# GavinLynch04/FastSelect

Hardware: AMD Instinct MI355X
Metric: feature-scores/sec (n*p/s) MultiSURF fp32 (higher is better)
Workload: dtype u16 pass 1, fp32 pass 2 (fp64 accumulation)

## Files before the change

fastselect_amd/csrc/fs_colsort.hip:

```cpp
#include <hip/hip_runtime.h>

#include <cstdlib>

#include <rocprim/block/block_radix_sort.hpp>
#include <rocprim/device/device_segmented_radix_sort.hpp>

#include "fs_internal.h"

namespace fs {
namespace gpu {

namespace {

constexpr double kEpsFx = 16777216.0;
constexpr int kCsThreads = 1024;
constexpr int kCsMaxIpt = 24;

__device__ __forceinline__ uint32_t cs_col_q(const uint32_t* __restrict__ xqT, int64_t c,
                                             int64_t i, int64_t n_pad, int q16) {
  return q16 ? (xqT[(c >> 1) * n_pad + i] >> ((c & 1) * 16)) & 0xFFFFu : xqT[c * n_pad + i];
}

__device__ __forceinline__ int32_t cs_fx(float eps) { return __float2int_rn(eps * 16777216.0f); }

__device__ __forceinline__ uint32_t cs_key(uint32_t q, int32_t fx, int s) {
  const uint32_t fr = (uint32_t)(((1 << 23) - fx) >> (24 - s));
  const uint32_t m = (1u << s) - 1u;
  return (q << s) | (fr < m ? fr : m);
}

__device__ __forceinline__ float cs_term(long long e, long long pos, long long n, long long P,
                                         long long T) {
  return (float)((double)(e * (2 * pos - n) - 2 * P + T) / kEpsFx);
}

__device__ __forceinline__ uint32_t cs_eq12_of_fx(int32_t fx) {
  const int32_t u = fx + (1 << 23);
  return (uint32_t)(u < 0 ? 0 : (u >= (1 << 24) ? 4095 : (u >> 12)));
}

__device__ __forceinline__ long long cs_block_scan(long long v, long long* wsum,
                                                   long long& total) {
  const int lane = threadIdx.x & 63, wave = threadIdx.x >> 6;
  long long x = v;
#pragma unroll
  for (int o = 1; o < 64; o <<= 1) {
    const long long t = __shfl_up(x, o);
    if (lane >= o) x += t;
  }
  if (lane == 63) wsum[wave] = x;
  __syncthreads();
  long long pre = 0, tot = 0;
#pragma unroll
  for (int w = 0; w < kCsThreads / 64; w++) {
    const long long s = wsum[w];
    pre += w < wave ? s : 0;
    tot += s;
  }
  __syncthreads();
  total = tot;
  return pre + x - v;
}

constexpr int kHistShift = 44;
constexpr int kMaxBinFill = 64;
constexpr uint32_t kPureEmpty = 0x7FFFFFFFu, kMixed = 0x80000000u;

__device__ __forceinline__ unsigned long long cs_code(int32_t fx) {
  return (1ull << kHistShift) + (unsigned long long)(uint32_t)(fx + (1 << 23));
}
__device__ __forceinline__ void cs_decode(unsigned long long v, long long& cnt, long long& esum) {
  cnt = (long long)(v >> kHistShift);
  esum = (long long)(v & ((1ull << kHistShift) - 1ull)) - (cnt << 23);
}

template <int IPT>
__global__ __launch_bounds__(kCsThreads) void k_colsort_full(const uint32_t* __restrict__ xqT,
                                                             int64_t n, int64_t n_pad, int s,
                                                             int q16, int64_t c_lo,
                                                             const int* __restrict__ crowded,
                                                             float* __restrict__ epsT) {
  using Sort = rocprim::block_radix_sort<uint32_t, kCsThreads, IPT, uint16_t>;
  __shared__ typename Sort::storage_type st;
  __shared__ long long wsum[kCsThreads / 64];
  if (!crowded[blockIdx.x]) return;
  const int64_t c = c_lo + blockIdx.x;
  float* __restrict__ e = epsT + c * n_pad;
  const int base = threadIdx.x * IPT;
  uint32_t key[IPT];
  uint16_t idx[IPT];
#pragma unroll
  for (int k = 0; k < IPT; k++) {
    const int i = base + k;
    key[k] = i < n ? cs_key(cs_col_q(xqT, c, i, n_pad, q16), cs_fx(e[i]), s) : 0xFFFFFFFFu;
    idx[k] = (uint16_t)i;
  }
  Sort().sort(key, idx, st);
  long long ef[IPT], loc = 0;
#pragma unroll
  for (int k = 0; k < IPT; k++) {
    ef[k] = base + k < n ? cs_fx(e[idx[k]]) : 0;
    loc += ef[k];
  }
  long long T;
  long long P = cs_block_scan(loc, wsum, T);
#pragma unroll
  for (int k = 0; k < IPT; k++) {
    const int pos = base + k;
    if (pos < n) e[idx[k]] = cs_term(ef[k], pos, n, P, T);
    P += ef[k];
  }
}

template <int IPT, int BB>
struct ColbinSmem {
  static constexpr int kBins = 1 << BB;
  unsigned long long hist[kBins];
  alignas(16) uint32_t seg[(kCsThreads * IPT > kBins ? kCsThreads * IPT : kBins) + 4];
  uint32_t starts[(kCsThreads * IPT + 31) / 32];
  uint32_t skip[(kCsThreads * IPT + 31) / 32];
  uint32_t binskip[kBins / 32];
  long long wsum[kCsThreads / 64];
  int max_fill;
};

#define FS_OPAQUE(v) asm volatile("" : "+v"(v))

__device__ __forceinline__ int32_t cs_pack(int d, int ds) { return ds * 256 + (d + 128); }
__device__ __forceinline__ void cs_unpack(int32_t r, int& d, int& ds) {
  d = (r & 255) - 128;
  ds = r >> 8;
}

template <int IPT, int BB>
__global__ __launch_bounds__(kCsThreads) void k_colsort(const uint32_t* __restrict__ xqT,
                                                        int64_t n, int64_t n_pad, int s, int q16,
                                                        int64_t c_lo, int* __restrict__ crowded,
                                                        float* __restrict__ epsT) {
  __shared__ ColbinSmem<IPT, BB> sm;
  constexpr int kBins = 1 << BB, kBinShift = 32 - BB;
  constexpr int kWords = (kCsThreads * IPT + 31) / 32;
  static_assert(sizeof(ColbinSmem<IPT, BB>) <= 160 * 1024, "k_colsort: LDS");
  const int tid = threadIdx.x;
  const int64_t c = c_lo + blockIdx.x;
  float* __restrict__ e = epsT + c * n_pad;
  const int nn = (int)n;
  uint32_t key[IPT];
  int32_t fx[IPT];
  for (int b = tid; b < kBins; b += kCsThreads) {
    sm.hist[b] = 0ull;
    sm.seg[b] = kPureEmpty;
  }
  for (int w = tid; w < kWords; w += kCsThreads) {
    sm.starts[w] = 0u;
    sm.skip[w] = 0u;
  }
  if (tid < kBins / 32) sm.binskip[tid] = 0u;
  if (tid == 0) sm.max_fill = 0;
  const __amdgpu_buffer_rsrc_t qbuf = __builtin_amdgcn_make_buffer_rsrc(
      (void*)(xqT + (q16 ? (c >> 1) : c) * n_pad), (short)0, nn * 4, 0x00020000);
  const __amdgpu_buffer_rsrc_t ebuf =
      __builtin_amdgcn_make_buffer_rsrc((void*)e, (short)0, nn * 4, 0x00020000);
  const int voff = tid * 4;
  const uint32_t qsh = q16 ? (uint32_t)(c & 1) * 16u : 0u;
  const uint32_t qmask = q16 ? 0xFFFFu : 0xFFFFFFFFu;
#pragma unroll
  for (int k = 0; k < IPT; k++) {
    key[k] = __builtin_amdgcn_raw_buffer_load_b32(qbuf, voff, kCsThreads * 4 * k, 0);
    fx[k] = (int32_t)__builtin_amdgcn_raw_buffer_load_b32(ebuf, voff, kCsThreads * 4 * k, 0);
  }
#pragma unroll
  for (int k = 0; k < IPT; k++) {
    fx[k] = cs_fx(__int_as_float(fx[k]));
    key[k] = cs_key((key[k] >> qsh) & qmask, fx[k], s);
  }
  __syncthreads();
#pragma unroll
  for (int k = 0; k < IPT; k++) {
    if (tid + kCsThreads * k >= nn) continue;
    const int b = (int)(key[k] >> kBinShift);
    atomicAdd(&sm.hist[b], cs_code(fx[k]));
    const uint32_t kl = key[k] & ((1u << kBinShift) - 1u);
    const uint32_t old = atomicCAS(&sm.seg[b], kPureEmpty, kl);
    if (old != kPureEmpty && (old & ((1u << kBinShift) - 1u)) != kl) atomicOr(&sm.seg[b], kMixed);
  }
  __syncthreads();
  constexpr int kPer = kBins / kCsThreads;
  unsigned long long run = 0;
  uint32_t skip_bits = 0;
  int fill = 0;
#pragma unroll
  for (int q = 0; q < kPer; q++) {
    const unsigned long long v = sm.hist[tid * kPer + q];
    const bool mixed = (sm.seg[tid * kPer + q] & kMixed) != 0u;
    run += v;
    if (mixed) fill = max(fill, (int)(v >> kHistShift));
    else skip_bits |= 1u << q;
  }
  long long tot_packed;
  const unsigned long long pre = (unsigned long long)cs_block_scan((long long)run, sm.wsum, tot_packed);
  unsigned long long ex = pre;
#pragma unroll 1
  for (int q = 0; q < kPer; q++) {
    const unsigned long long v = sm.hist[tid * kPer + q];
    const uint32_t lo = (uint32_t)(ex >> kHistShift);
    const uint32_t m = (uint32_t)(v >> kHistShift);
    const bool skip = ((skip_bits >> q) & 1u) != 0u;
    sm.hist[tid * kPer + q] = ex;
    ex += v;
    if (m != 0u) {
      atomicOr(&sm.starts[lo >> 5], 1u << (lo & 31));
      if (skip) {
        const uint32_t hi = lo + m;
        for (uint32_t w = lo >> 5; w <= (hi - 1) >> 5; w++) {
          const uint32_t a = w == (lo >> 5) ? (lo & 31) : 0u;
          const uint32_t z = w == ((hi - 1) >> 5) ? ((hi - 1) & 31) : 31u;
          const uint32_t bits = (0xFFFFFFFFu >> (31u - z)) & (0xFFFFFFFFu << a);
          atomicOr(&sm.skip[w], bits);
        }
      }
    }
  }
  atomicOr(&sm.binskip[(tid * kPer) >> 5], skip_bits << ((tid * kPer) & 31));
  atomicMax(&sm.max_fill, fill);
  __syncthreads();
  const bool crowd = sm.max_fill > kMaxBinFill;
  if (tid == 0) crowded[blockIdx.x] = crowd ? 1 : 0;
  if (crowd) return;
  long long n_all, T;
  cs_decode((unsigned long long)tot_packed, n_all, T);
  int t3 = tid;
  FS_OPAQUE(t3);
#pragma unroll
  for (int k = 0; k < IPT; k++) {
    FS_OPAQUE(key[k]);
    FS_OPAQUE(fx[k]);
    const uint32_t b = key[k] >> kBinShift;
    uint32_t pos = 0xFFFFu;
    if (t3 + kCsThreads * k < nn) {
      const uint32_t at = (uint32_t)(atomicAdd(&sm.hist[b], 1ull << kHistShift) >> kHistShift);
      if (!((sm.binskip[b >> 5] >> (b & 31)) & 1u)) {
        pos = at;
        sm.seg[pos] = ((key[k] & ((1u << kBinShift) - 1u)) << 12) | cs_eq12_of_fx(fx[k]);
      }
    }
    key[k] = (b << 16) | pos;
    FS_OPAQUE(key[k]);
    __builtin_amdgcn_sched_barrier(0);
  }
  __syncthreads();
  int32_t res[IPT];
  int t4 = tid;
  FS_OPAQUE(t4);
#pragma unroll
  for (int k = 0; k < IPT; k++) {
    const int j = t4 + kCsThreads * k;
    res[k] = 0;
    if (j >= nn || ((sm.skip[j >> 5] >> (j & 31)) & 1u)) continue;
    int w = j >> 5;
    uint32_t bits = sm.starts[w] & (0xFFFFFFFFu >> (31 - (j & 31)));
    while (bits == 0u) bits = sm.starts[--w];
    const int lo = w * 32 + 31 - __clz(bits);
    int hi = nn;
    w = j >> 5;
    bits = (j & 31) == 31 ? 0u : sm.starts[w] & (0xFFFFFFFFu << ((j & 31) + 1));
    while (bits == 0u && ++w < kWords && w * 32 < nn) bits = sm.starts[w];
    if (bits != 0u) hi = min(nn, w * 32 + __ffs(bits) - 1);
    const uint32_t v = sm.seg[j];
    const uint32_t mine_lo = v & ~0xFFFu, mine_hi = v | 0xFFFu;
    uint32_t a_lt = 0u, a_le = 0u, a_all = 0u;
    for (int jj = lo; jj < hi; jj++) {
      const uint32_t u = sm.seg[jj];
      const uint32_t wv = (u & 0xFFFu) | (1u << 20);
      a_lt += u < mine_lo ? wv : 0u;
      a_le += u <= mine_hi ? wv : 0u;
      a_all += wv;
    }
    const int l = (int)(a_lt >> 20), sl = (int)(a_lt & 0xFFFFFu);
    const int g = (int)(a_all >> 20) - (int)(a_le >> 20);
    const int sg = (int)(a_all & 0xFFFFFu) - (int)(a_le & 0xFFFFFu);
    res[k] = cs_pack(l - g, sl - sg);
    __builtin_amdgcn_sched_barrier(0);
  }
  __syncthreads();
#pragma unroll
  for (int k = 0; k < IPT; k++) {
    const int j = t4 + kCsThreads * k;
    if (j < nn && !((sm.skip[j >> 5] >> (j & 31)) & 1u)) sm.seg[j] = (uint32_t)res[k];
  }
  __syncthreads();
#pragma unroll
  for (int k = 0; k < IPT; k++)
    fx[k] = (int32_t)__builtin_amdgcn_raw_buffer_load_b32(ebuf, voff, kCsThreads * 4 * k, 0);
  int t5 = tid;
  FS_OPAQUE(t5);
#pragma unroll
  for (int k = 0; k < IPT; k++) {
    FS_OPAQUE(key[k]);
    const int i = t5 + kCsThreads * k;
    if (i >= nn) continue;
    const int32_t f = cs_fx(__int_as_float(fx[k]));
    const int b = (int)(key[k] >> 16);
    constexpr unsigned long long kLow = (1ull << kHistShift) - 1ull;
    const unsigned long long here = sm.hist[b];
    const unsigned long long above = b + 1 < kBins ? sm.hist[b + 1] : (unsigned long long)tot_packed;
    const long long c_below = b ? (long long)(sm.hist[b - 1] >> kHistShift) : 0ll;
    const long long c_to = (long long)(here >> kHistShift);
    const long long e_below = (long long)(here & kLow) - (c_below << 23);
    const long long e_to = (long long)(above & kLow) - (c_to << 23);
    long long dLG = c_below - (nn - c_to), dE = e_below - (T - e_to);
    const uint32_t pos = key[k] & 0xFFFFu;
    if (pos != 0xFFFFu) {
      int d, ds;
      cs_unpack((int32_t)sm.seg[pos], d, ds);
      dLG += d;
      dE += (long long)(2 * ds + d) * 2048 - (long long)d * (1ll << 23);
    }
    const float term = (float)((double)((long long)f * dLG - dE) * (1.0 / kEpsFx));
    __builtin_amdgcn_raw_buffer_store_b32(__float_as_uint(term), ebuf, voff, kCsThreads * 4 * k, 0);
    __builtin_amdgcn_sched_barrier(0);
  }
}

__global__ __launch_bounds__(256) void k_colsort_keys(const uint32_t* __restrict__ xqT, int64_t n,
                                                      int64_t n_pad, int s, int q16, int64_t c0,
                                                      const float* __restrict__ epsT,
                                                      uint32_t* __restrict__ keys,
                                                      uint32_t* __restrict__ vals) {
  const int64_t cc = blockIdx.y;
  const int64_t i = (int64_t)blockIdx.x * 256 + threadIdx.x;
  if (i >= n) return;
  const int64_t c = c0 + cc;
  keys[cc * n + i] = cs_key(cs_col_q(xqT, c, i, n_pad, q16), cs_fx(epsT[c * n_pad + i]), s);
  vals[cc * n + i] = (uint32_t)i;
}

constexpr int kScanIpt = 8;
__global__ __launch_bounds__(kCsThreads) void k_colsort_scan(const uint32_t* __restrict__ vals,
                                                             int64_t n, int64_t n_pad, int64_t c0,
                                                             float* __restrict__ epsT) {
  __shared__ long long wsum[kCsThreads / 64];
  const int64_t cc = blockIdx.x;
  float* __restrict__ e = epsT + (c0 + cc) * n_pad;
  const uint32_t* __restrict__ v = vals + cc * n;
  long long loc = 0;
  for (int64_t i = threadIdx.x; i < n; i += kCsThreads) loc += cs_fx(e[i]);
  long long T;
  (void)cs_block_scan(loc, wsum, T);
  long long carry = 0;
  for (int64_t b = 0; b < n; b += (int64_t)kCsThreads * kScanIpt) {
    const int64_t base = b + (int64_t)threadIdx.x * kScanIpt;
    uint32_t id[kScanIpt];
    long long ef[kScanIpt], sum = 0;
#pragma unroll
    for (int k = 0; k < kScanIpt; k++) {
      const bool in = base + k < n;
      id[k] = in ? v[base + k] : 0u;
      ef[k] = in ? cs_fx(e[id[k]]) : 0;
      sum += ef[k];
    }
    long long chunk;
    long long P = carry + cs_block_scan(sum, wsum, chunk);
#pragma unroll
    for (int k = 0; k < kScanIpt; k++) {
      if (base + k < n) e[id[k]] = cs_term(ef[k], base + k, n, P, T);
      P += ef[k];
    }
    carry += chunk;
  }
}

__global__ void k_colsort_offsets(int64_t n, int64_t nc, unsigned* __restrict__ off) {
  const int64_t k = (int64_t)blockIdx.x * blockDim.x + threadIdx.x;
  if (k <= nc) off[k] = (unsigned)(k * n);
}

__device__ __forceinline__ void cs_scan2(double& a, double& b, double (*ws)[kCsThreads / 64],
                                         double& ta, double& tb) {
  const int lane = threadIdx.x & 63, wave = threadIdx.x >> 6;
  double x = a, y = b;
#pragma unroll
  for (int o = 1; o < 64; o <<= 1) {
    const double tx = __shfl_up(x, o), ty = __shfl_up(y, o);
    if (lane >= o) {
      x += tx;
      y += ty;
    }
  }
  if (lane == 63) {
    ws[0][wave] = x;
    ws[1][wave] = y;
  }
  __syncthreads();
  double pa = 0.0, pb = 0.0, sa = 0.0, sb = 0.0;
#pragma unroll
  for (int w = 0; w < kCsThreads / 64; w++) {
    const double u = ws[0][w], v = ws[1][w];
    if (w < wave) {
      pa += u;
      pb += v;
    }
    sa += u;
    sb += v;
  }
  __syncthreads();
  ta = sa;
  tb = sb;
  a = pa + x - a;
  b = pb + y - b;
}

template <int IPT>
__global__ __launch_bounds__(kCsThreads) void k_colsort_star(
    const uint32_t* __restrict__ xqT, int64_t n, int64_t n_pad, int s, int q16, int64_t c_lo,
    float* __restrict__ epsT, float* __restrict__ xsT, const int32_t* __restrict__ lab,
    const int64_t* __restrict__ out_pos, int ncls) {
  using Sort = rocprim::block_radix_sort<uint32_t, kCsThreads, IPT, uint16_t>;
  __shared__ typename Sort::storage_type st;
  __shared__ long long wsum[kCsThreads / 64];
  __shared__ double ws2[2][kCsThreads / 64];
  const int64_t c = c_lo + blockIdx.x;
  float* __restrict__ e = epsT + c * n_pad;
  float* __restrict__ xv = xsT + c * n_pad;
  const int base = threadIdx.x * IPT;
  uint32_t key[IPT];
  uint16_t idx[IPT];
#pragma unroll
  for (int k = 0; k < IPT; k++) {
    const int i = base + k;
    key[k] = i < n ? cs_key(cs_col_q(xqT, c, i, n_pad, q16), cs_fx(e[i]), s) : 0xFFFFFFFFu;
    idx[k] = (uint16_t)i;
  }
  Sort().sort(key, idx, st);
  long long ef[IPT], loc = 0;
#pragma unroll
  for (int k = 0; k < IPT; k++) {
    ef[k] = base + k < n ? cs_fx(e[idx[k]]) : 0;
    loc += ef[k];
  }
  long long T;
  long long P = cs_block_scan(loc, wsum, T);
#pragma unroll
  for (int k = 0; k < IPT; k++) {
    const int pos = base + k;
    if (pos < n) e[idx[k]] = cs_term(ef[k], pos, n, P, T);
    P += ef[k];
  }
  if (out_pos[c] < 0) return;
  float v[IPT], so[IPT];
  int cl[IPT];
#pragma unroll
  for (int k = 0; k < IPT; k++) {
    const bool ok = base + k < n;
    v[k] = ok ? xv[idx[k]] : 0.0f;
    cl[k] = ok ? lab[idx[k]] : -1;
    so[k] = 0.0f;
  }
  for (int q = 0; q < ncls; q++) {
    double lc = 0.0, ls = 0.0;
#pragma unroll
    for (int k = 0; k < IPT; k++)
      if (cl[k] == q) {
        lc += 1.0;
        ls += (double)v[k];
      }
    double tc, ts;
    cs_scan2(lc, ls, ws2, tc, ts);
#pragma unroll
    for (int k = 0; k < IPT; k++) {
      const double vk = (double)v[k];
      if (cl[k] >= 0 && cl[k] != q) so[k] += (float)(vk * (2.0 * lc - tc) - 2.0 * ls + ts);
      if (cl[k] == q) {
        lc += 1.0;
        ls += vk;
      }
    }
  }
#pragma unroll
  for (int k = 0; k < IPT; k++)
    if (base + k < n) xv[idx[k]] = so[k];
}

int64_t batch_cols(int64_t n, int64_t ncols) {
  int64_t b = std::max<int64_t>(1, ((int64_t)512 << 20) / (16 * std::max<int64_t>(n, 1)));
  b = std::min<int64_t>(b, 4096);
  return std::min<int64_t>(b, std::max<int64_t>(ncols, 1));
}

size_t align256(size_t b) { return (b + 255) & ~(size_t)255; }

size_t batch_bytes(int64_t n, int64_t nb) {
  return 4 * align256(sizeof(uint32_t) * (size_t)(n * nb)) + align256(sizeof(unsigned) * (nb + 1));
}

}

int colsort_bin_bits(int64_t n) {
  const bool force12 = test_hooks().colsort_bins12 != 0;
  return !force12 && n > 12 * (int64_t)kCsThreads && n <= 20 * (int64_t)kCsThreads ? 13 : 12;
}

bool colsort_lds(int64_t n) {
  return !test_hooks().colsort_global && n <= (int64_t)kCsThreads * kCsMaxIpt;
}

size_t colsort_scratch_bytes(int64_t n, int64_t ncols) {
  if (ncols <= 0) return 0;
  if (colsort_lds(n)) return align256(sizeof(int) * (size_t)ncols);
  const int64_t nb = batch_cols(n, ncols);
  if ((unsigned long long)n * nb >= (1ull << 32)) return 0;
  size_t temp = 0;
  uint32_t* nk = nullptr;
  unsigned* no = nullptr;
  if (rocprim::segmented_radix_sort_pairs(nullptr, temp, nk, nk, nk, nk, (unsigned)(n * nb),
                                          (unsigned)nb, no, no + 1, 0, 32) != hipSuccess) {
    (void)hipGetLastError();
    return 0;
  }
  return batch_bytes(n, nb) + align256(temp);
}

int colsort_star_terms(const uint32_t* xqT, float* epsT, float* xsT, const int32_t* lab,
                       const int64_t* out_pos, int ncls, int64_t n, int64_t n_pad, int64_t c_lo,
                       int64_t c_hi, int q16, int key_shift, void* stream_v) {
  hipStream_t stream = (hipStream_t)stream_v;
  const int64_t nc = c_hi - c_lo;
  if (nc <= 0 || n < 1) return 0;
  if (n > (int64_t)kCsThreads * kCsMaxIpt) {
    set_error("k_colsort_star: more samples than one workgroup sorts");
    return -1;
  }
  const unsigned grid = (unsigned)nc;
#define FS_CSS(IPT)                                                                            \
  k_colsort_star<IPT><<<grid, kCsThreads, 0, stream>>>(xqT, n, n_pad, key_shift, q16, c_lo,     \
                                                       epsT, xsT, lab, out_pos, ncls)
  const int64_t ipt = (n + kCsThreads - 1) / kCsThreads;
  if (ipt <= 4) FS_CSS(4);
  else if (ipt <= 8) FS_CSS(8);
  else if (ipt <= 10) FS_CSS(10);
  else if (ipt <= 12) FS_CSS(12);
  else if (ipt <= 16) FS_CSS(16);
  else if (ipt <= 20) FS_CSS(20);
  else FS_CSS(24);
#undef FS_CSS
  if (hipGetLastError() != hipSuccess) {
    set_error("k_colsort_star: launch failed");
    return -1;
  }
  return 0;
}

int colsort_terms(const uint32_t* xqT, float* epsT, int64_t n, int64_t n_pad, int64_t c_lo,
                  int64_t c_hi, int q16, int key_shift, void* scratch, size_t scratch_bytes,
                  void* stream_v) {
  hipStream_t stream = (hipStream_t)stream_v;
  const int64_t nc = c_hi - c_lo;
  if (nc <= 0 || n < 1) return 0;
  if (colsort_lds(n)) {
    int* crowded = (int*)scratch;
    if (!crowded || scratch_bytes < sizeof(int) * (size_t)nc) {
      set_error("k_colsort: scratch too small for the column flags");
      return -1;
    }
    const unsigned grid = (unsigned)nc;
#define FS_COLSORT(IPT, BB)                                                                      \
  do {                                                                                           \
    k_colsort<IPT, BB><<<grid, kCsThreads, 0, stream>>>(xqT, n, n_pad, key_shift, q16, c_lo,      \
                                                        crowded, epsT);                          \
    k_colsort_full<IPT><<<grid, kCsThreads, 0, stream>>>(xqT, n, n_pad, key_shift, q16, c_lo,     \
                                                         crowded, epsT);                          \
  } while (0)
    const int64_t ipt = (n + kCsThreads - 1) / kCsThreads;
    const bool b13 = colsort_bin_bits(n) == 13;
    if (ipt <= 2) FS_COLSORT(2, 12);
    else if (ipt <= 4) FS_COLSORT(4, 12);
    else if (ipt <= 5) FS_COLSORT(5, 12);
    else if (ipt <= 6) FS_COLSORT(6, 12);
    else if (ipt <= 8) FS_COLSORT(8, 12);
    else if (ipt <= 10) FS_COLSORT(10, 12);
    else if (ipt <= 12) FS_COLSORT(12, 12);
    else if (ipt <= 16 && b13) FS_COLSORT(16, 13);
    else if (ipt <= 16) FS_COLSORT(16, 12);
    else if (ipt <= 20 && b13) FS_COLSORT(20, 13);
    else if (ipt <= 20) FS_COLSORT(20, 12);
    else FS_COLSORT(24, 12);
#undef FS_COLSORT
    if (hipGetLastError() != hipSuccess) {
      set_error("k_colsort: launch failed");
      return -1;
    }
    return 0;
  }
  const int64_t nb = batch_cols(n, nc);
  const size_t need = colsort_scratch_bytes(n, nc);
  if (need == 0 || scratch_bytes < need || !scratch) {
    set_error("k_colsort: scratch too small for the large-n route");
    return -1;
  }
  char* p = (char*)scratch;
  const size_t kb = align256(sizeof(uint32_t) * (size_t)(n * nb));
  uint32_t* k_in = (uint32_t*)p;
  uint32_t* k_out = (uint32_t*)(p + kb);
  uint32_t* v_in = (uint32_t*)(p + 2 * kb);
  uint32_t* v_out = (uint32_t*)(p + 3 * kb);
  unsigned* off = (unsigned*)(p + 4 * kb);
  void* temp = p + batch_bytes(n, nb);
  size_t temp_bytes = scratch_bytes - batch_bytes(n, nb);
  for (int64_t c0 = c_lo; c0 < c_hi; c0 += nb) {
    const int64_t m = std::min<int64_t>(nb, c_hi - c0);
    k_colsort_offsets<<<(unsigned)((m + 256) / 256), 256, 0, stream>>>(n, m, off);
    k_colsort_keys<<<dim3((unsigned)((n + 255) / 256), (unsigned)m), 256, 0, stream>>>(
        xqT, n, n_pad, key_shift, q16, c0, epsT, k_in, v_in);
    if (hipGetLastError() != hipSuccess) {
      set_error("k_colsort_keys: launch failed");
      return -1;
    }
    if (rocprim::segmented_radix_sort_pairs(temp, temp_bytes, k_in, k_out, v_in, v_out,
                                            (unsigned)(n * m), (unsigned)m, off, off + 1, 0, 32,
                                            stream) != hipSuccess) {
      (void)hipGetLastError();
      set_error("k_colsort: segmented radix sort failed");
      return -1;
    }
    k_colsort_scan<<<(unsigned)m, kCsThreads, 0, stream>>>(v_out, n, n_pad, c0, epsT);
    if (hipGetLastError() != hipSuccess) {
      set_error("k_colsort_scan: launch failed");
      return -1;
    }
  }
  return 0;
}

}
}
```

Before: 2.927 billion.

## Make column-sort kernel persistent with per-CU grid and tighter within-bin walk

Turns k_colsort into a persistent kernel: the grid is capped at one workgroup per CU and each workgroup loops over columns, issuing the next column's global loads before clearing shared memory. The within-bin comparison loop becomes a single signed accumulator walked in unrolled chunks, and the block scan uses ds_bpermute directly. Shared-memory init is limited to the words actually used. Optional wall-clock phase profiling is added behind a macro. The intent is to cut launch and workgroup-setup overhead and to shorten the inner compare loop. The risk is less latency hiding when only one workgroup runs per CU.

```diff
diff --git a/fastselect_amd/csrc/fs_colsort.hip b/fastselect_amd/csrc/fs_colsort.hip
--- a/fastselect_amd/csrc/fs_colsort.hip
+++ b/fastselect_amd/csrc/fs_colsort.hip
@@ -1,6 +1,8 @@
 #include <hip/hip_runtime.h>
 
+#include <cstdio>
 #include <cstdlib>
+#include <vector>
 
 #include <rocprim/block/block_radix_sort.hpp>
 #include <rocprim/device/device_segmented_radix_sort.hpp>
@@ -40,12 +42,15 @@
 }
 
 __device__ __forceinline__ long long cs_block_scan(long long v, long long* wsum,
-                                                   long long& total) {
-  const int lane = threadIdx.x & 63, wave = threadIdx.x >> 6;
+                                                   long long& total, int tid) {
+  const int lane = tid & 63, wave = tid >> 6;
   long long x = v;
 #pragma unroll
   for (int o = 1; o < 64; o <<= 1) {
-    const long long t = __shfl_up(x, o);
+    const int src = ((lane - o) & 63) << 2;
+    const uint32_t tl = (uint32_t)__builtin_amdgcn_ds_bpermute(src, (int)(uint32_t)x);
+    const uint32_t th = (uint32_t)__builtin_amdgcn_ds_bpermute(src, (int)((unsigned long long)x >> 32));
+    const long long t = (long long)(((unsigned long long)th << 32) | tl);
     if (lane >= o) x += t;
   }
   if (lane == 63) wsum[wave] = x;
@@ -66,9 +71,6 @@
 constexpr int kMaxBinFill = 64;
 constexpr uint32_t kPureEmpty = 0x7FFFFFFFu, kMixed = 0x80000000u;
 
-__device__ __forceinline__ unsigned long long cs_code(int32_t fx) {
-  return (1ull << kHistShift) + (unsigned long long)(uint32_t)(fx + (1 << 23));
-}
 __device__ __forceinline__ void cs_decode(unsigned long long v, long long& cnt, long long& esum) {
   cnt = (long long)(v >> kHistShift);
   esum = (long long)(v & ((1ull << kHistShift) - 1ull)) - (cnt << 23);
@@ -103,7 +105,7 @@
     loc += ef[k];
   }
   long long T;
-  long long P = cs_block_scan(loc, wsum, T);
+  long long P = cs_block_scan(loc, wsum, T, (int)threadIdx.x);
 #pragma unroll
   for (int k = 0; k < IPT; k++) {
     const int pos = base + k;
@@ -117,7 +119,7 @@
   static constexpr int kBins = 1 << BB;
   unsigned long long hist[kBins];
   alignas(16) uint32_t seg[(kCsThreads * IPT > kBins ? kCsThreads * IPT : kBins) + 4];
-  uint32_t starts[(kCsThreads * IPT + 31) / 32];
+  uint32_t starts[(kCsThreads * IPT + 31) / 32 + 2];
   uint32_t skip[(kCsThreads * IPT + 31) / 32];
   uint32_t binskip[kBins / 32];
   long long wsum[kCsThreads / 64];
@@ -127,198 +129,290 @@
 #define FS_OPAQUE(v) asm volatile("" : "+v"(v))
 
 __device__ __forceinline__ int32_t cs_pack(int d, int ds) { return ds * 256 + (d + 128); }
+constexpr int32_t kNoCounts = INT32_MIN;
 __device__ __forceinline__ void cs_unpack(int32_t r, int& d, int& ds) {
   d = (r & 255) - 128;
   ds = r >> 8;
 }
 
+[[maybe_unused]] constexpr int kProfSlots = 8;
+
+#ifndef FS_CS_GROUP
+#define FS_CS_GROUP 2
+#endif
+constexpr int kCsGroup = FS_CS_GROUP;
+#ifndef FS_CS_WALK
+#define FS_CS_WALK 4
+#endif
+constexpr int kCsWalk = FS_CS_WALK;
+#ifndef FS_CS_WG_PER_CU
+#define FS_CS_WG_PER_CU 1
+#endif
+constexpr int64_t kCsWgPerCu = FS_CS_WG_PER_CU;
+#ifdef FS_CS_PROF
+#define FS_CS_STAMP(slot)                                 \
+  do {                                                    \
+    __builtin_amdgcn_sched_barrier(0);                    \
+    const unsigned long long t_now = wall_clock64();      \
+    if (tid == 0) prof[slot] = t_now - t_prev;            \
+    t_prev = t_now;                                       \
+    __builtin_amdgcn_sched_barrier(0);                    \
+  } while (0)
+#else
+#define FS_CS_STAMP(slot) \
+  do {                    \
+  } while (0)
+#endif
+
 template <int IPT, int BB>
 __global__ __launch_bounds__(kCsThreads) void k_colsort(const uint32_t* __restrict__ xqT,
                                                         int64_t n, int64_t n_pad, int s, int q16,
-                                                        int64_t c_lo, int* __restrict__ crowded,
+                                                        int64_t c_lo, int nc,
+                                                        int* __restrict__ crowded,
                                                         float* __restrict__ epsT) {
   __shared__ ColbinSmem<IPT, BB> sm;
   constexpr int kBins = 1 << BB, kBinShift = 32 - BB;
-  constexpr int kWords = (kCsThreads * IPT + 31) / 32;
   static_assert(sizeof(ColbinSmem<IPT, BB>) <= 160 * 1024, "k_colsort: LDS");
   const int tid = threadIdx.x;
-  const int64_t c = c_lo + blockIdx.x;
-  float* __restrict__ e = epsT + c * n_pad;
   const int nn = (int)n;
+  const int words = (nn + 31) >> 5;
+#ifdef FS_CS_PROF
+  unsigned long long* const prof_base =
+      (unsigned long long*)((char*)crowded + (((size_t)nc * 4 + 255) & ~(size_t)255));
+  unsigned long long t_prev = wall_clock64();
+#endif
   uint32_t key[IPT];
   int32_t fx[IPT];
-  for (int b = tid; b < kBins; b += kCsThreads) {
-    sm.hist[b] = 0ull;
-    sm.seg[b] = kPureEmpty;
-  }
-  for (int w = tid; w < kWords; w += kCsThreads) {
-    sm.starts[w] = 0u;
-    sm.skip[w] = 0u;
-  }
-  if (tid < kBins / 32) sm.binskip[tid] = 0u;
-  if (tid == 0) sm.max_fill = 0;
-  const __amdgpu_buffer_rsrc_t qbuf = __builtin_amdgcn_make_buffer_rsrc(
-      (void*)(xqT + (q16 ? (c >> 1) : c) * n_pad), (short)0, nn * 4, 0x00020000);
-  const __amdgpu_buffer_rsrc_t ebuf =
-      __builtin_amdgcn_make_buffer_rsrc((void*)e, (short)0, nn * 4, 0x00020000);
-  const int voff = tid * 4;
-  const uint32_t qsh = q16 ? (uint32_t)(c & 1) * 16u : 0u;
   const uint32_t qmask = q16 ? 0xFFFFu : 0xFFFFFFFFu;
-#pragma unroll
-  for (int k = 0; k < IPT; k++) {
-    key[k] = __builtin_amdgcn_raw_buffer_load_b32(qbuf, voff, kCsThreads * 4 * k, 0);
-    fx[k] = (int32_t)__builtin_amdgcn_raw_buffer_load_b32(ebuf, voff, kCsThreads * 4 * k, 0);
-  }
-#pragma unroll
-  for (int k = 0; k < IPT; k++) {
-    fx[k] = cs_fx(__int_as_float(fx[k]));
-    key[k] = cs_key((key[k] >> qsh) & qmask, fx[k], s);
-  }
-  __syncthreads();
-#pragma unroll
-  for (int k = 0; k < IPT; k++) {
-    if (tid + kCsThreads * k >= nn) continue;
-    const int b = (int)(key[k] >> kBinShift);
-    atomicAdd(&sm.hist[b], cs_code(fx[k]));
-    const uint32_t kl = key[k] & ((1u << kBinShift) - 1u);
-    const uint32_t old = atomicCAS(&sm.seg[b], kPureEmpty, kl);
-    if (old != kPureEmpty && (old & ((1u << kBinShift) - 1u)) != kl) atomicOr(&sm.seg[b], kMixed);
-  }
-  __syncthreads();
-  constexpr int kPer = kBins / kCsThreads;
-  unsigned long long run = 0;
-  uint32_t skip_bits = 0;
-  int fill = 0;
-#pragma unroll
-  for (int q = 0; q < kPer; q++) {
-    const unsigned long long v = sm.hist[tid * kPer + q];
-    const bool mixed = (sm.seg[tid * kPer + q] & kMixed) != 0u;
-    run += v;
-    if (mixed) fill = max(fill, (int)(v >> kHistShift));
-    else skip_bits |= 1u << q;
-  }
-  long long tot_packed;
-  const unsigned long long pre = (unsigned long long)cs_block_scan((long long)run, sm.wsum, tot_packed);
-  unsigned long long ex = pre;
+  for (int cc = (int)blockIdx.x; cc < nc; cc += (int)gridDim.x) {
+    const int64_t c = c_lo + cc;
+    const __amdgpu_buffer_rsrc_t qbuf = __builtin_amdgcn_make_buffer_rsrc(
+        (void*)(xqT + (q16 ? (c >> 1) : c) * n_pad), (short)0, nn * 4, 0x00020000);
+    const __amdgpu_buffer_rsrc_t ebuf = __builtin_amdgcn_make_buffer_rsrc(
+        (void*)(epsT + c * n_pad), (short)0, nn * 4, 0x00020000);
+    int t0 = tid;
+    FS_OPAQUE(t0);
+#pragma unroll
+    for (int k = 0; k < IPT; k++) {
+      key[k] = __builtin_amdgcn_raw_buffer_load_b32(qbuf, t0 * 4, kCsThreads * 4 * k, 0);
+      fx[k] = (int32_t)__builtin_amdgcn_raw_buffer_load_b32(ebuf, t0 * 4, kCsThreads * 4 * k, 0);
+    }
+#ifdef FS_CS_PROF
+    unsigned long long* prof = prof_base + (size_t)cc * kProfSlots;
+    if (tid == 0) prof[kProfSlots - 1] = t_prev;
+#endif
+    __syncthreads();
+    {
+      uint32_t zero = 0u;
+      FS_OPAQUE(zero);
+      for (int b = t0; b < kBins; b += kCsThreads) {
+        sm.hist[b] = ((unsigned long long)zero << 32) | zero;
+        sm.seg[b] = kPureEmpty;
+      }
+      for (int w = t0; w < words + 2; w += kCsThreads) {
+        sm.starts[w] = 0u;
+        if (w < words) sm.skip[w] = 0u;
+      }
+      if (t0 < kBins / 32) sm.binskip[t0] = 0u;
+      if (t0 == 0) sm.max_fill = 0;
+    }
+    {
+      const uint32_t qsh = q16 ? (uint32_t)(c & 1) * 16u : 0u;
+#pragma unroll
+      for (int k = 0; k < IPT; k++) {
+        fx[k] = cs_fx(__int_as_float(fx[k]));
+        key[k] = cs_key((key[k] >> qsh) & qmask, fx[k], s);
+      }
+    }
+    __syncthreads();
+    FS_CS_STAMP(0);
+    int t1 = tid;
+    FS_OPAQUE(t1);
+#pragma unroll
+    for (int k = 0; k < IPT; k++) {
+      if (t1 + kCsThreads * k >= nn) continue;
+      const int b = (int)(key[k] >> kBinShift);
+      uint32_t one = 1u << (kHistShift - 32);
+      FS_OPAQUE(one);
+      atomicAdd(&sm.hist[b], ((unsigned long long)one << 32) | (uint32_t)(fx[k] + (1 << 23)));
+      const uint32_t kl = key[k] & ((1u << kBinShift) - 1u);
+      const uint32_t old = atomicCAS(&sm.seg[b], kPureEmpty, kl);
+      if (old != kPureEmpty && (old & ((1u << kBinShift) - 1u)) != kl) atomicOr(&sm.seg[b], kMixed);
+    }
+    __syncthreads();
+    FS_CS_STAMP(1);
+    constexpr int kPer = kBins / kCsThreads;
+    int t2 = tid;
+    FS_OPAQUE(t2);
+    unsigned long long run = 0;
+    uint32_t skip_bits = 0;
+    int fill = 0;
+#pragma unroll
+    for (int q = 0; q < kPer; q++) {
+      const unsigned long long v = sm.hist[t2 * kPer + q];
+      const bool mixed = (sm.seg[t2 * kPer + q] & kMixed) != 0u;
+      run += v;
+      if (mixed) fill = max(fill, (int)(v >> kHistShift));
+      else skip_bits |= 1u << q;
+    }
+    long long tot_packed;
+    const unsigned long long pre = (unsigned long long)cs_block_scan((long long)run, sm.wsum, tot_packed, t2);
+    tot_packed = (long long)(((unsigned long long)__builtin_amdgcn_readfirstlane(
+                                  (int)((unsigned long long)tot_packed >> 32))
+                              << 32) |
+                             (uint32_t)__builtin_amdgcn_readfirstlane((int)tot_packed));
+    unsigned long long ex = pre;
 #pragma unroll 1
-  for (int q = 0; q < kPer; q++) {
-    const unsigned long long v = sm.hist[tid * kPer + q];
-    const uint32_t lo = (uint32_t)(ex >> kHistShift);
-    const uint32_t m = (uint32_t)(v >> kHistShift);
-    const bool skip = ((skip_bits >> q) & 1u) != 0u;
-    sm.hist[tid * kPer + q] = ex;
-    ex += v;
-    if (m != 0u) {
-      atomicOr(&sm.starts[lo >> 5], 1u << (lo & 31));
-      if (skip) {
-        const uint32_t hi = lo + m;
-        for (uint32_t w = lo >> 5; w <= (hi - 1) >> 5; w++) {
-          const uint32_t a = w == (lo >> 5) ? (lo & 31) : 0u;
-          const uint32_t z = w == ((hi - 1) >> 5) ? ((hi - 1) & 31) : 31u;
-          const uint32_t bits = (0xFFFFFFFFu >> (31u - z)) & (0xFFFFFFFFu << a);
-          atomicOr(&sm.skip[w], bits);
+    for (int q = 0; q < kPer; q++) {
+      const unsigned long long v = sm.hist[t2 * kPer + q];
+      const uint32_t lo = (uint32_t)(ex >> kHistShift);
+      const uint32_t m = (uint32_t)(v >> kHistShift);
+      const bool skip = ((skip_bits >> q) & 1u) != 0u;
+      sm.hist[t2 * kPer + q] = ex;
+      ex += v;
+      if (m != 0u) {
+        atomicOr(&sm.starts[lo >> 5], 1u << (lo & 31));
+        if (skip) {
+          const uint32_t hi = lo + m;
+          for (uint32_t w = lo >> 5; w <= (hi - 1) >> 5; w++) {
+            const uint32_t a = w == (lo >> 5) ? (lo & 31) : 0u;
+            const uint32_t z = w == ((hi - 1) >> 5) ? ((hi - 1) & 31) : 31u;
+            const uint32_t bits = (0xFFFFFFFFu >> (31u - z)) & (0xFFFFFFFFu << a);
+            atomicOr(&sm.skip[w], bits);
+          }
         }
       }
     }
-  }
-  atomicOr(&sm.binskip[(tid * kPer) >> 5], skip_bits << ((tid * kPer) & 31));
-  atomicMax(&sm.max_fill, fill);
-  __syncthreads();
-  const bool crowd = sm.max_fill > kMaxBinFill;
-  if (tid == 0) crowded[blockIdx.x] = crowd ? 1 : 0;
-  if (crowd) return;
-  long long n_all, T;
-  cs_decode((unsigned long long)tot_packed, n_all, T);
-  int t3 = tid;
-  FS_OPAQUE(t3);
-#pragma unroll
-  for (int k = 0; k < IPT; k++) {
-    FS_OPAQUE(key[k]);
-    FS_OPAQUE(fx[k]);
-    const uint32_t b = key[k] >> kBinShift;
-    uint32_t pos = 0xFFFFu;
-    if (t3 + kCsThreads * k < nn) {
-      const uint32_t at = (uint32_t)(atomicAdd(&sm.hist[b], 1ull << kHistShift) >> kHistShift);
-      if (!((sm.binskip[b >> 5] >> (b & 31)) & 1u)) {
-        pos = at;
-        sm.seg[pos] = ((key[k] & ((1u << kBinShift) - 1u)) << 12) | cs_eq12_of_fx(fx[k]);
-      }
-    }
-    key[k] = (b << 16) | pos;
-    FS_OPAQUE(key[k]);
-    __builtin_amdgcn_sched_barrier(0);
-  }
-  __syncthreads();
-  int32_t res[IPT];
-  int t4 = tid;
-  FS_OPAQUE(t4);
-#pragma unroll
-  for (int k = 0; k < IPT; k++) {
-    const int j = t4 + kCsThreads * k;
-    res[k] = 0;
-    if (j >= nn || ((sm.skip[j >> 5] >> (j & 31)) & 1u)) continue;
-    int w = j >> 5;
-    uint32_t bits = sm.starts[w] & (0xFFFFFFFFu >> (31 - (j & 31)));
-    while (bits == 0u) bits = sm.starts[--w];
-    const int lo = w * 32 + 31 - __clz(bits);
-    int hi = nn;
-    w = j >> 5;
-    bits = (j & 31) == 31 ? 0u : sm.starts[w] & (0xFFFFFFFFu << ((j & 31) + 1));
-    while (bits == 0u && ++w < kWords && w * 32 < nn) bits = sm.starts[w];
-    if (bits != 0u) hi = min(nn, w * 32 + __ffs(bits) - 1);
-    const uint32_t v = sm.seg[j];
-    const uint32_t mine_lo = v & ~0xFFFu, mine_hi = v | 0xFFFu;
-    uint32_t a_lt = 0u, a_le = 0u, a_all = 0u;
-    for (int jj = lo; jj < hi; jj++) {
-      const uint32_t u = sm.seg[jj];
-      const uint32_t wv = (u & 0xFFFu) | (1u << 20);
-      a_lt += u < mine_lo ? wv : 0u;
-      a_le += u <= mine_hi ? wv : 0u;
-      a_all += wv;
-    }
-    const int l = (int)(a_lt >> 20), sl = (int)(a_lt & 0xFFFFFu);
-    const int g = (int)(a_all >> 20) - (int)(a_le >> 20);
-    const int sg = (int)(a_all & 0xFFFFFu) - (int)(a_le & 0xFFFFFu);
-    res[k] = cs_pack(l - g, sl - sg);
-    __builtin_amdgcn_sched_barrier(0);
-  }
-  __syncthreads();
-#pragma unroll
-  for (int k = 0; k < IPT; k++) {
-    const int j = t4 + kCsThreads * k;
-    if (j < nn && !((sm.skip[j >> 5] >> (j & 31)) & 1u)) sm.seg[j] = (uint32_t)res[k];
-  }
-  __syncthreads();
-#pragma unroll
-  for (int k = 0; k < IPT; k++)
-    fx[k] = (int32_t)__builtin_amdgcn_raw_buffer_load_b32(ebuf, voff, kCsThreads * 4 * k, 0);
-  int t5 = tid;
-  FS_OPAQUE(t5);
-#pragma unroll
-  for (int k = 0; k < IPT; k++) {
-    FS_OPAQUE(key[k]);
-    const int i = t5 + kCsThreads * k;
-    if (i >= nn) continue;
-    const int32_t f = cs_fx(__int_as_float(fx[k]));
-    const int b = (int)(key[k] >> 16);
-    constexpr unsigned long long kLow = (1ull << kHistShift) - 1ull;
-    const unsigned long long here = sm.hist[b];
-    const unsigned long long above = b + 1 < kBins ? sm.hist[b + 1] : (unsigned long long)tot_packed;
-    const long long c_below = b ? (long long)(sm.hist[b - 1] >> kHistShift) : 0ll;
-    const long long c_to = (long long)(here >> kHistShift);
-    const long long e_below = (long long)(here & kLow) - (c_below << 23);
-    const long long e_to = (long long)(above & kLow) - (c_to << 23);
-    long long dLG = c_below - (nn - c_to), dE = e_below - (T - e_to);
-    const uint32_t pos = key[k] & 0xFFFFu;
-    if (pos != 0xFFFFu) {
-      int d, ds;
-      cs_unpack((int32_t)sm.seg[pos], d, ds);
-      dLG += d;
-      dE += (long long)(2 * ds + d) * 2048 - (long long)d * (1ll << 23);
-    }
-    const float term = (float)((double)((long long)f * dLG - dE) * (1.0 / kEpsFx));
-    __builtin_amdgcn_raw_buffer_store_b32(__float_as_uint(term), ebuf, voff, kCsThreads * 4 * k, 0);
-    __builtin_amdgcn_sched_barrier(0);
+    atomicOr(&sm.binskip[(t2 * kPer) >> 5], skip_bits << ((t2 * kPer) & 31));
+    atomicMax(&sm.max_fill, fill);
+    __syncthreads();
+    FS_CS_STAMP(2);
+    const bool crowd = sm.max_fill > kMaxBinFill;
+    if (tid == 0) crowded[cc] = crowd ? 1 : 0;
+    if (!crowd) {
+      long long n_all, T;
+      cs_decode((unsigned long long)tot_packed, n_all, T);
+      int t3 = tid;
+      FS_OPAQUE(t3);
+#pragma unroll
+      for (int k = 0; k < IPT; k++) {
+        FS_OPAQUE(key[k]);
+        FS_OPAQUE(fx[k]);
+        const uint32_t b = key[k] >> kBinShift;
+        uint32_t pos = 0xFFFFu;
+        if (t3 + kCsThreads * k < nn) {
+          uint32_t one = 1u << (kHistShift - 32);
+          FS_OPAQUE(one);
+          const uint32_t at =
+              (uint32_t)(atomicAdd(&sm.hist[b], (unsigned long long)one << 32) >> kHistShift);
+          if (!((sm.binskip[b >> 5] >> (b & 31)) & 1u)) {
+            pos = at;
+            sm.seg[pos] = ((key[k] & ((1u << kBinShift) - 1u)) << 12) | cs_eq12_of_fx(fx[k]);
+          }
+        }
+        key[k] = (b << 16) | pos;
+        FS_OPAQUE(key[k]);
+        if (k % kCsGroup == kCsGroup - 1) __builtin_amdgcn_sched_barrier(0);
+      }
+      __syncthreads();
+      FS_CS_STAMP(3);
+      int32_t res[IPT];
+      int t4 = tid;
+      FS_OPAQUE(t4);
+#pragma unroll
+      for (int k = 0; k < IPT; k++) {
+        const int j = t4 + kCsThreads * k;
+        res[k] = kNoCounts;
+        if (j >= nn || ((sm.skip[j >> 5] >> (j & 31)) & 1u)) continue;
+        const int w = j >> 5, r = j & 31;
+        uint32_t s0 = sm.starts[w];
+        uint32_t sb1 = sm.starts[max(w - 1, 0)], sb2 = sm.starts[max(w - 2, 0)];
+        uint32_t sa1 = sm.starts[w + 1], sa2 = sm.starts[w + 2];
+        const uint32_t v = sm.seg[j];
+        FS_OPAQUE(s0);
+        FS_OPAQUE(sb1);
+        FS_OPAQUE(sb2);
+        FS_OPAQUE(sa1);
+        FS_OPAQUE(sa2);
+        const uint32_t b0 = s0 & (0xFFFFFFFFu >> (31 - r));
+        const int lo = b0 ? w * 32 + 31 - __clz(b0)
+                          : (sb1 ? (w - 1) * 32 + 31 - __clz(sb1) : (w - 2) * 32 + 31 - __clz(sb2));
+        const uint32_t a0 = r == 31 ? 0u : s0 & (0xFFFFFFFFu << (r + 1));
+        const int hi = a0 ? w * 32 + __ffs(a0) - 1
+                          : (sa1 ? (w + 1) * 32 + __ffs(sa1) - 1
+                                 : (sa2 ? (w + 2) * 32 + __ffs(sa2) - 1 : nn));
+        const int mine = (int)(v >> 12);
+        int acc = 0;
+        int jj = lo;
+#pragma unroll 1
+        for (; jj + kCsWalk <= hi; jj += kCsWalk) {
+          uint32_t u[kCsWalk];
+#pragma unroll
+          for (int q = 0; q < kCsWalk; q++) u[q] = sm.seg[jj + q];
+#pragma unroll
+          for (int q = 0; q < kCsWalk; q++) {
+            const int sgn = min(max(mine - (int)(u[q] >> 12), -1), 1);
+            acc += sgn * (int)((u[q] & 0xFFFu) | (1u << 20));
+          }
+        }
+        if (jj < hi) {
+          uint32_t u[kCsWalk];
+#pragma unroll
+          for (int q = 0; q < kCsWalk - 1; q++) u[q] = sm.seg[jj + q];
+#pragma unroll
+          for (int q = 0; q < kCsWalk - 1; q++) {
+            const int sgn = jj + q < hi ? min(max(mine - (int)(u[q] >> 12), -1), 1) : 0;
+            acc += sgn * (int)((u[q] & 0xFFFu) | (1u << 20));
+          }
+        }
+        const int ds = ((acc + (1 << 19)) & 0xFFFFF) - (1 << 19);
+        res[k] = cs_pack((acc - ds) >> 20, ds);
+        __builtin_amdgcn_sched_barrier(0);
+      }
+      __syncthreads();
+      FS_CS_STAMP(4);
+      int t4s = tid;
+      FS_OPAQUE(t4s);
+#pragma unroll
+      for (int k = 0; k < IPT; k++)
+        if (res[k] != kNoCounts) sm.seg[t4s + kCsThreads * k] = (uint32_t)res[k];
+      __syncthreads();
+      FS_CS_STAMP(5);
+      int t5 = tid;
+      FS_OPAQUE(t5);
+#pragma unroll
+      for (int k = 0; k < IPT; k++)
+        fx[k] = (int32_t)__builtin_amdgcn_raw_buffer_load_b32(ebuf, t5 * 4, kCsThreads * 4 * k, 0);
+#pragma unroll
+      for (int k = 0; k < IPT; k++) {
+        FS_OPAQUE(key[k]);
+        FS_OPAQUE(fx[k]);
+        const int i = t5 + kCsThreads * k;
+        if (i < nn) {
+          const int32_t f = cs_fx(__int_as_float(fx[k]));
+          const int b = (int)(key[k] >> 16);
+          constexpr unsigned long long kLow = (1ull << kHistShift) - 1ull;
+          const unsigned long long here = sm.hist[b];
+          const unsigned long long above = b + 1 < kBins ? sm.hist[b + 1] : (unsigned long long)tot_packed;
+          const long long c_below = b ? (long long)(sm.hist[b - 1] >> kHistShift) : 0ll;
+          const long long c_to = (long long)(here >> kHistShift);
+          const long long e_below = (long long)(here & kLow) - (c_below << 23);
+          const long long e_to = (long long)(above & kLow) - (c_to << 23);
+          long long dLG = c_below - (nn - c_to), dE = e_below - (T - e_to);
+          const uint32_t pos = key[k] & 0xFFFFu;
+          if (pos != 0xFFFFu) {
+            int d, ds;
+            cs_unpack((int32_t)sm.seg[pos], d, ds);
+            dLG += d;
+            dE += (long long)(2 * ds + d) * 2048 - (long long)d * (1ll << 23);
+          }
+          const float term = (float)((double)((long long)f * dLG - dE) * (1.0 / kEpsFx));
+          __builtin_amdgcn_raw_buffer_store_b32(__float_as_uint(term), ebuf, t5 * 4, kCsThreads * 4 * k, 0);
+        }
+        if (k % kCsGroup == kCsGroup - 1) __builtin_amdgcn_sched_barrier(0);
+      }
+    }
+    FS_CS_STAMP(6);
   }
 }
 
@@ -346,7 +440,7 @@
   long long loc = 0;
   for (int64_t i = threadIdx.x; i < n; i += kCsThreads) loc += cs_fx(e[i]);
   long long T;
-  (void)cs_block_scan(loc, wsum, T);
+  (void)cs_block_scan(loc, wsum, T, (int)threadIdx.x);
   long long carry = 0;
   for (int64_t b = 0; b < n; b += (int64_t)kCsThreads * kScanIpt) {
     const int64_t base = b + (int64_t)threadIdx.x * kScanIpt;
@@ -360,7 +454,7 @@
       sum += ef[k];
     }
     long long chunk;
-    long long P = carry + cs_block_scan(sum, wsum, chunk);
+    long long P = carry + cs_block_scan(sum, wsum, chunk, (int)threadIdx.x);
 #pragma unroll
     for (int k = 0; k < kScanIpt; k++) {
       if (base + k < n) e[id[k]] = cs_term(ef[k], base + k, n, P, T);
@@ -439,7 +533,7 @@
     loc += ef[k];
   }
   long long T;
-  long long P = cs_block_scan(loc, wsum, T);
+  long long P = cs_block_scan(loc, wsum, T, (int)threadIdx.x);
 #pragma unroll
   for (int k = 0; k < IPT; k++) {
     const int pos = base + k;
@@ -493,6 +587,44 @@
   return 4 * align256(sizeof(uint32_t) * (size_t)(n * nb)) + align256(sizeof(unsigned) * (nb + 1));
 }
 
+#ifdef FS_CS_PROF
+void cs_prof_report(const int* crowded, int64_t nc, int64_t n, unsigned grid, hipStream_t stream) {
+  std::vector<unsigned long long> h((size_t)(kProfSlots * nc));
+  std::vector<int> cr((size_t)nc);
+  const char* prof = (const char*)crowded + align256(sizeof(int) * (size_t)nc);
+  if (hipStreamSynchronize(stream) != hipSuccess ||
+      hipMemcpy(cr.data(), crowded, sizeof(int) * nc, hipMemcpyDeviceToHost) != hipSuccess ||
+      hipMemcpy(h.data(), prof, sizeof(unsigned long long) * h.size(), hipMemcpyDeviceToHost) !=
+          hipSuccess) {
+    (void)hipGetLastError();
+    return;
+  }
+  double sum[kProfSlots - 1] = {}, all = 0.0;
+  unsigned long long t0 = ~0ull, t1 = 0ull;
+  int64_t m = 0;
+  for (int64_t c = 0; c < nc; c++) {
+    const unsigned long long* r = &h[(size_t)(c * kProfSlots)];
+    unsigned long long end = r[kProfSlots - 1];
+    for (int k = 0; k < kProfSlots - 1; k++) end += r[k];
+    t0 = std::min(t0, r[kProfSlots - 1]);
+    t1 = std::max(t1, end);
+    if (cr[(size_t)c]) continue;
+    m++;
+    for (int k = 0; k < kProfSlots - 1; k++) sum[k] += 0.01 * (double)r[k];
+  }
+  for (double& v : sum) {
+    v /= (double)std::max<int64_t>(m, 1);
+    all += v;
+  }
+  fprintf(stderr,
+          "k_colsort phases: n %lld, columns %lld (binned %lld), workgroups %u; us per column: "
+          "load+init %.2f, (1) count %.2f, (2) scan %.2f, (3) scatter %.2f, (4) within-bin %.2f, "
+          "store counts %.2f, (5) terms %.2f, sum %.2f; first entry to last exit %.1f us\n",
+          (long long)n, (long long)nc, (long long)m, grid, sum[0], sum[1], sum[2], sum[3], sum[4],
+          sum[5], sum[6], all, 0.01 * (double)(t1 - t0));
+}
+#endif
+
 }
 
 int colsort_bin_bits(int64_t n) {
@@ -506,7 +638,13 @@
 
 size_t colsort_scratch_bytes(int64_t n, int64_t ncols) {
   if (ncols <= 0) return 0;
-  if (colsort_lds(n)) return align256(sizeof(int) * (size_t)ncols);
+  if (colsort_lds(n)) {
+    size_t b = align256(sizeof(int) * (size_t)ncols);
+#ifdef FS_CS_PROF
+    b += sizeof(unsigned long long) * kProfSlots * (size_t)ncols;
+#endif
+    return b;
+  }
   const int64_t nb = batch_cols(n, ncols);
   if ((unsigned long long)n * nb >= (1ull << 32)) return 0;
   size_t temp = 0;
@@ -558,17 +696,30 @@
   if (nc <= 0 || n < 1) return 0;
   if (colsort_lds(n)) {
     int* crowded = (int*)scratch;
-    if (!crowded || scratch_bytes < sizeof(int) * (size_t)nc) {
+    if (!crowded || scratch_bytes < colsort_scratch_bytes(n, nc)) {
       set_error("k_colsort: scratch too small for the column flags");
       return -1;
     }
-    const unsigned grid = (unsigned)nc;
+    if (nc > INT32_MAX) {
+      set_error("k_colsort: too many columns");
+      return -1;
+    }
+    int dev = 0, cus = 0;
+    if (hipGetDevice(&dev) != hipSuccess ||
+        hipDeviceGetAttribute(&cus, hipDeviceAttributeMultiprocessorCount, dev) != hipSuccess ||
+        cus < 1) {
+      (void)hipGetLastError();
+      set_error("k_colsort: no compute unit count");
+      return -1;
+    }
+    const unsigned grid_full = (unsigned)nc;
+    const unsigned grid = (unsigned)std::min<int64_t>(nc, (int64_t)cus * kCsWgPerCu);
 #define FS_COLSORT(IPT, BB)                                                                      \
   do {                                                                                           \
     k_colsort<IPT, BB><<<grid, kCsThreads, 0, stream>>>(xqT, n, n_pad, key_shift, q16, c_lo,      \
-                                                        crowded, epsT);                          \
-    k_colsort_full<IPT><<<grid, kCsThreads, 0, stream>>>(xqT, n, n_pad, key_shift, q16, c_lo,     \
-                                                         crowded, epsT);                          \
+                                                        (int)nc, crowded, epsT);                 \
+    k_colsort_full<IPT><<<grid_full, kCsThreads, 0, stream>>>(xqT, n, n_pad, key_shift, q16,      \
+                                                              c_lo, crowded, epsT);               \
   } while (0)
     const int64_t ipt = (n + kCsThreads - 1) / kCsThreads;
     const bool b13 = colsort_bin_bits(n) == 13;
@@ -589,6 +740,9 @@
       set_error("k_colsort: launch failed");
       return -1;
     }
+#ifdef FS_CS_PROF
+    cs_prof_report(crowded, nc, n, grid, stream);
+#endif
     return 0;
   }
   const int64_t nb = batch_cols(n, nc);
```

Result: no change. 2.929 billion (median of 5 runs) (+0.1%).
